# soniareilly/HPCClassMultigridProject

Measured on AMD Instinct MI355X. Metric: V-cycle grid-point-updates/sec at N=16384; achieved HBM GB/s vs peak, higher is better.
Workload: dtype f64

## Files before the change

hpcclassmultigridproject_amd/csrc/kernels.h:

```cpp
#pragma once
#include <hip/hip_runtime.h>

namespace mgx {

struct Coef {
    double rr, nu, h, dgs, drhs, rdgs;
    unsigned dsign;
    double g, gn, c2;
    int fm;
};
Coef make_coef(double k, double nu, double h, int fm = 0);

long tower_pitch(long n);

void launch_raw_gs_colour(double *u, const double *rhs, const double *v1, const double *v2,
                          long n, Coef c, int colour, hipStream_t s);
void launch_raw_residual(double *res, const double *u, const double *rhs, const double *v1,
                         const double *v2, long n, Coef c, hipStream_t s);
void launch_raw_rhs(double *rhs, const double *u, const double *v1, const double *v2, long n,
                    Coef c, hipStream_t s);
void launch_raw_prolongation(double *up, const double *u, long n, hipStream_t s);
void launch_injection(double *dst, long dst_pitch, const double *src, long src_pitch, long m,
                      hipStream_t s);
void launch_injection_rows(double *dst, long dst_pitch, const double *src, long src_pitch,
// ... 25 lines not shown
constexpr int kCoarseLdsMaxN = 64;
constexpr int kCoarseLdsNP = kCoarseLdsMaxN + 1;

struct CoarseFuse {
    double *u = nullptr;
    const double *rhs = nullptr, *v1 = nullptr, *v2 = nullptr;
    long n = 0, pitch = 0;
    Coef c{};
    double tol = 0.0;
    int maxit = 0, zero_first = 0, reps = 0;
    double *stats = nullptr;
    int on = 0;
};

struct SmoothArgs {
    const double *uin;
    double *uout;
    const double *rhs, *v1, *v2;
    long n, pitch;
    Coef c;
    const double *uc;
    double *rhsc;
    long pitchc;
    double *partials;
    double *norm_out;
    double *rhs_out = nullptr;
    const double *zrow = nullptr;
    int vz = 0x7fffffff;
    VGen vg{};
    bool norm_sqrt = true;
    bool norm_accumulate = false;
    int ra = 0, rb = -1, lo = 0, hi = -1;
    CoarseFuse cf{};
};
int launch_smooth(const SmoothArgs &a, int sweeps, int mode, hipStream_t s);
int launch_smooth_wpair(const SmoothArgs &a, int nsmooth, hipStream_t s);
bool smooth_generates_velocity(const SmoothArgs &a, int sweeps, int mode);

struct XArgs {
    const double *uin = nullptr;
    double *upost = nullptr, *upre = nullptr;
    const double *rhs = nullptr, *v1 = nullptr, *v2 = nullptr;
    const double *uc = nullptr;
    long pitchc = 0;
    double *rhsc = nullptr;
    double *partials = nullptr, *norm_out = nullptr;
    long n = 0, pitch = 0;
    Coef c{};
    bool store_post = true;
    bool norm_sqrt = true;
    bool norm_accumulate = false;
    int ra = 0, rb = -1, lo = 0, hi = -1;
    int min_rows = 64;
    double *rhs_next = nullptr, *norm2_out = nullptr;
    const double *sa1 = nullptr, *sb1 = nullptr, *sa2 = nullptr, *sb2 = nullptr;
    int band = 0, phase = 0, partials_done = 0;
    bool pin = false, pout = false;
};
int launch_xsmooth(const XArgs &a, int sweeps, hipStream_t s);
bool xpack_supported(long n, double dgs);
void launch_xexpand(const XArgs &a, const double *packed, double *out, hipStream_t s);
bool xstep_supported(long n);
void set_xfast(long v);
long get_xfast();
void set_march_tile_rows(long v);
long get_march_tile_rows();
void set_xtile_max_rows(long v);
long get_xtile_max_rows();
// ... 39 lines not shown
```

hpcclassmultigridproject_amd/csrc/mgx.hip:

```cpp
#include <hip/hip_runtime.h>

#include <algorithm>
#include <cmath>
#include <cstdint>
#include <cstdio>
#include <cstring>
#include <mutex>
#include <string>
#include <vector>

#include "ctx.h"
#include "diag.h"
#include "sepvel.h"
#include "source.h"
#include "vfactor.h"

namespace mgxi {

thread_local std::string g_err;

long g_sep_velocity = 1;

bool factor_velocity(const double *v1, const double *v2, long n, long r0, long rows, double smin,
                     std::vector<double> &a1, std::vector<double> &b1, std::vector<double> &a2,
// ... 78 lines not shown
    return MGX_OK;
}

hipEvent_t take_event(mgx_ctx *c) {
    if (!c->pool.empty()) {
        hipEvent_t e = c->pool.back();
        c->pool.pop_back();
        return e;
    }
    hipEvent_t e = nullptr;
    if (hipEventCreate(&e) != hipSuccess) return nullptr;
    return e;
}

int prof_flush(mgx_ctx *c) {
    if (c->pending.empty()) return MGX_OK;
    HIPCHK(hipStreamSynchronize(c->stream));
    for (auto &r : c->pending) {
        float ms = 0.f;
        HIPCHK(hipEventSynchronize(r.e1));
        HIPCHK(hipEventElapsedTime(&ms, r.e0, r.e1));
        int lvl = r.level < 0 ? 0 : (r.level > 63 ? 63 : r.level);
        c->sum_ms[r.kind][lvl] += ms;
        c->sum_bytes[r.kind][lvl] += r.bytes;
        c->sum_cbytes[r.kind][lvl] += r.cbytes;
        c->count[r.kind][lvl] += 1;
        c->pool.push_back(r.e0);
        c->pool.push_back(r.e1);
    }
    c->pending.clear();
    return MGX_OK;
}

int materialize(mgx_ctx *c, int l) {
    Level &L = c->lv[l];
    if (!L.zero) return MGX_OK;
    HIPCHK(hipMemsetAsync(L.U(), 0, sizeof(double) * L.pitch * (L.n + 1), c->stream));
    L.zero = false;
    return MGX_OK;
}

int op_prolong_add(mgx_ctx *c, int l);
int op_restrict(mgx_ctx *c, int l);
long g_vgen = 1;
static mgx::VGen level_vgen(const mgx_ctx *c, int l) {
    mgx::VGen g;
    g.a = c->vga;
    g.b1 = c->lv[0].sb1;
    g.b2 = c->lv[0].sb2;
    g.l = l;
    g.strided = c->opt.tower_mode == MGX_TOWER_CORRECT ? 1 : 0;
    return g;
}
long g_coarse_fuse = 1;
int op_coarse(mgx_ctx *c, int l, int reps);
static bool coarse_fusable(const mgx_ctx *c, int l) {
    return g_coarse_fuse && !c->dist && c->opt.smoother == 0 && c->opt.nsmooth >= 1 &&
           l == c->L - 1 && l >= 2 && c->lv[l].zero &&
           c->lv[l].n <= mgx::kCoarseLdsMaxN && mgx::get_coarse_lds() &&
           c->lv[l - 1].n <= mgx::get_tile_max_n();
}
static int flush_coarse(mgx_ctx *c) {
    if (c->cf_level < 0) return MGX_OK;
    const int l = c->cf_level;
    c->cf_level = -1;
    return op_coarse(c, l, c->cf_reps);
}
static int check_coarse_rhs(const mgx::SmoothArgs &A, int mode) {
    if (A.cf.on && (mode & mgx::kModeRestrict) && A.rhsc == A.cf.rhs)
        return fail(MGX_E_INTERNAL, "fused coarsest solve reads the rhs its pass restricts into");
    return MGX_OK;
}
static bool take_coarse(mgx_ctx *c, int l, mgx::SmoothArgs &A) {
    if (c->cf_level != l + 1) return false;
    Level &Cl = c->lv[l + 1];
    A.cf.u = Cl.U();
    A.cf.rhs = Cl.rhs;
    A.cf.v1 = Cl.v1;
    A.cf.v2 = Cl.v2;
    A.cf.n = Cl.n;
    A.cf.pitch = Cl.pitch;
    A.cf.c = Cl.coef;
    A.cf.tol = c->opt.coarse_tol;
    A.cf.maxit = c->opt.coarse_maxit;
    A.cf.zero_first = Cl.zero ? 1 : 0;
    A.cf.reps = c->cf_reps;
    A.cf.stats = c->dscal + 2;
    A.cf.on = 1;
    return true;
}
static void took_coarse(mgx_ctx *c, int l) {
    c->cf_level = -1;
    c->lv[l + 1].zero = false;
}

int op_smooth(mgx_ctx *c, int l, int sweeps, bool prolong, bool restrict_, bool norm,
              bool *fused_norm) {
    Level &L = c->lv[l];
    if (fused_norm) *fused_norm = false;
    if (c->opt.smoother == 0 && sweeps > 0) {
        const int fuse = std::max(1, std::min(c->opt.fuse, mgx::kSmoothMaxSweeps));
        int done = 0;
        while (done < sweeps) {
            const int k = std::min(sweeps - done, fuse);
            const bool first = done == 0, last = done + k == sweeps;
            const bool pr = prolong && first && !L.zero;
            const bool rs = restrict_ && last;
            const bool nm = norm && last && !rs;
            const bool cfuse = pr && c->cf_level == l + 1;
            if (pr && !cfuse) CHK(materialize(c, l + 1));
            int mode = 0;
            if (L.zero) mode |= mgx::kModeZero;
            if (pr) mode |= mgx::kModeProlong;
            if (rs) mode |= mgx::kModeRestrict;
            if (nm) mode |= mgx::kModeNorm;
            mgx::SmoothArgs A{};
            A.uin = L.u[L.cur];
            A.uout = L.u[L.nxt()];
            A.rhs = L.rhs;
            A.v1 = L.v1;
            A.v2 = L.v2;
            A.zrow = c->zrow;
            A.vz = L.vz;
            if (L.vgen && g_vgen) A.vg = level_vgen(c, l);
            A.n = L.n;
            A.pitch = L.pitch;
            A.c = L.coef;
            if (pr || rs) {
                Level &Cl = c->lv[l + 1];
                A.uc = Cl.U();
                A.rhsc = Cl.rhs;
                A.pitchc = Cl.pitch;
            }
            A.partials = c->partials;
            A.norm_out = c->dscal;
            if (cfuse) take_coarse(c, l, A);
            double bytes = 40.0 * k * L.M();
            int kind = MGX_K_GS;
            if (pr) {
                bytes += 32.0 * L.M() + 8.0 * c->lv[l + 1].M();
                kind = MGX_K_PSMOOTH;
            }
            if (rs) bytes += 40.0 * L.M() + 24.0 * c->lv[l + 1].M();
            if (nm) bytes += 48.0 * L.M();
            const bool vgu = mgx::smooth_generates_velocity(A, k, mode);
            const double cbytes = 8.0 * (((mode & mgx::kModeZero) ? 2.0 : 3.0) * L.M() +
                                         (vgu ? 0.0 : 2.0 * L.Mv()) +
                                         ((pr ? 1 : 0) + (rs ? 1 : 0)) * c->lv[l + 1].M());
            int blocks = 0;
            CHK(check_coarse_rhs(A, mode));
            const size_t before = c->pending.size();
            CHK(launch(c, kind, l, bytes, cbytes,
                       [&] { blocks = mgx::launch_smooth(A, k, mode, c->stream); }));
            if (blocks < 0) unlaunch(c, before);
            if (blocks == -4 && cfuse) {
                A.cf = mgx::CoarseFuse{};
                CHK(flush_coarse(c));
                A.uc = c->lv[l + 1].U();
                CHK(launch(c, kind, l, bytes, cbytes,
                           [&] { blocks = mgx::launch_smooth(A, k, mode, c->stream); }));
            } else if (cfuse) {
                took_coarse(c, l);
            }
            if (blocks < 0) return fail(MGX_E_ARG, "launch_smooth: unsupported sweeps/mode");
            L.cur = L.nxt();
            L.packed[L.cur] = false;
            L.zero = false;
            if (rs) c->lv[l + 1].zero = true;
            if (nm && fused_norm) *fused_norm = true;
            done += k;
        }
        if (prolong && L.zero) CHK(op_prolong_add(c, l));
        return MGX_OK;
    }
    if (prolong) CHK(op_prolong_add(c, l));
    for (int k = 0; k < sweeps; ++k) {
        if (c->opt.smoother == 2) {
            const bool z = L.zero;
            CHK(launch(c, MGX_K_GS, l, 40.0 * L.M(), [&] {
                mgx::launch_gs_sweep(L.u[L.cur], L.u[L.nxt()], L.rhs, L.v1, L.v2, L.n, L.pitch,
                                     L.coef, z, c->stream);
            }));
            L.cur = L.nxt();
            L.zero = false;
        } else {
            CHK(materialize(c, l));
            CHK(launch(c, MGX_K_GS, l, 40.0 * L.M(), [&] {
                mgx::launch_gs_colour(L.U(), L.rhs, L.v1, L.v2, L.n, L.pitch, L.coef, 0,
                                      c->stream);
                mgx::launch_gs_colour(L.U(), L.rhs, L.v1, L.v2, L.n, L.pitch, L.coef, 1,
                                      c->stream);
            }));
        }
    }
    if (restrict_) CHK(op_restrict(c, l));
    return MGX_OK;
}

int op_gs(mgx_ctx *c, int l, int sweeps) {
// ... 16 lines not shown
    }));
    return read_norm(c, norm);
}

int op_restrict(mgx_ctx *c, int l) {
    CHK(materialize(c, l));
    Level &F = c->lv[l], &C = c->lv[l + 1];
    CHK(launch(c, MGX_K_RESTRICT, l, 40.0 * F.M() + 24.0 * C.M(), 32.0 * F.M() + 8.0 * C.M(), [&] {
        mgx::launch_residual_restrict(F.U(), F.rhs, F.v1, F.v2, F.n, F.pitch, F.coef, C.rhs,
                                      C.pitch, c->stream);
    }));
    C.zero = true;
    return MGX_OK;
}

int op_prolong_add(mgx_ctx *c, int l) {
    CHK(flush_coarse(c));
    CHK(materialize(c, l));
    CHK(materialize(c, l + 1));
    Level &F = c->lv[l], &C = c->lv[l + 1];
    CHK(launch(c, MGX_K_PROLONG, l, 32.0 * F.M() + 8.0 * C.M(), 16.0 * F.M() + 8.0 * C.M(), [&] {
        mgx::launch_prolong_add(F.U(), F.pitch, C.U(), C.pitch, C.n, c->stream);
    }));
    return MGX_OK;
}

long g_wpair = 1;
int op_wpair(mgx_ctx *c, int l, bool *done) {
    *done = false;
    Level &L = c->lv[l], &Cl = c->lv[l + 1];
    const int k = c->opt.nsmooth;
    if (!g_wpair || c->opt.smoother != 0 || k < 1 || k > 3 || c->opt.fuse < k || L.zero)
        return MGX_OK;
    if (c->cf_level == l + 1 && !Cl.rhs_alt) CHK(flush_coarse(c));
    const bool cfuse = c->cf_level == l + 1;
    if (Cl.zero && !cfuse) return MGX_OK;
    mgx::SmoothArgs A{};
    A.uin = L.u[L.cur];
    A.uout = L.u[L.nxt()];
    A.rhs = L.rhs;
    A.v1 = L.v1;
    A.v2 = L.v2;
    A.n = L.n;
    A.pitch = L.pitch;
    A.c = L.coef;
    A.uc = Cl.U();
    A.rhsc = cfuse ? Cl.rhs_alt : Cl.rhs;
    A.pitchc = Cl.pitch;
    A.partials = c->partials;
    A.norm_out = c->dscal;
    if (cfuse) take_coarse(c, l, A);
    CHK(check_coarse_rhs(A, mgx::kModeProlong | mgx::kModeRestrict));
    const double bytes = (32.0 + 40.0 * k) * L.M() + 8.0 * Cl.M() + (40.0 * k + 40.0) * L.M() +
                         24.0 * Cl.M();
    const double cbytes = 8.0 * (3.0 * L.M() + 2.0 * L.Mv() + 2.0 * Cl.M());
    int blocks = 0;
    const size_t before = c->pending.size();
    CHK(launch(c, MGX_K_PSMOOTH, l, bytes, cbytes,
               [&] { blocks = mgx::launch_smooth_wpair(A, k, c->stream); }));
    if (blocks < 0) unlaunch(c, before);
    if (blocks == -4) return flush_coarse(c);
    if (blocks < 0) return MGX_OK;
    if (cfuse) {
        took_coarse(c, l);
        std::swap(Cl.rhs, Cl.rhs_alt);
    }
// ... 227 lines not shown
                                  c->stream));
            HIPCHK(hipMemcpyAsync(c->hscal + 6, c->dscal + 6, sizeof(double),
                                  hipMemcpyDeviceToHost, c->stream));
            HIPCHK(hipStreamSynchronize(c->stream));
            *norm = c->hscal[0];
            c->step_res0 = c->hscal[6];
            c->step_spec = true;
            return MGX_OK;
        }
        if (c->post_only) {
            bool fused = false;
            CHK(op_expand(c));
            CHK(op_smooth(c, 0, c->opt.nsmooth, true, false, true, &fused));
            L.spec = -1;
            return fused ? read_norm(c, norm) : op_residual_norm(c, 0, norm);
        }
        CHK(op_cross(c, store_post));
        return read_norm(c, norm);
    }
    if (l == 0) drop_spec(c);
    bool have_norm = false;
    bool pre_done = false;
    for (int sh = 0; sh < (l == c->L - 1 ? 1 : c->opt.shape); ++sh) {
        const bool last = sh == c->opt.shape - 1;
        if (l == c->L - 1) {
            if (coarse_fusable(c, l)) {
                c->cf_level = l;
                c->cf_reps = c->opt.shape;
            } else {
                CHK(op_coarse(c, l, c->opt.shape));
            }
        } else {
            if (!pre_done)
                CHK(op_smooth(c, l, c->opt.nsmooth, false, true, false, nullptr));
            pre_done = false;
            CHK(op_vcycle(c, l + 1));
            if (!last) {
                bool fused = false;
                CHK(op_wpair(c, l, &fused));
                if (fused) {
                    pre_done = true;
                    continue;
                }
            }
            CHK(op_smooth(c, l, c->opt.nsmooth, true, false, norm && last,
                          &have_norm));
            CHK(flush_coarse(c));
        }
    }
    if (norm) {
        if (have_norm)
            CHK(read_norm(c, norm));
        else
            CHK(op_residual_norm(c, l, norm));
    }
    return MGX_OK;
}

long g_source_sv = 1;

static mgxsrc::SrcArgs source_args(mgx_ctx *c, bool norm, double *cbytes) {
    Level &L = c->lv[0];
    mgxsrc::SrcArgs A;
    A.rhs = L.rhs;
    A.u = L.U();
    A.v1 = L.v1;
    A.v2 = L.v2;
// ... 1404 lines not shown
        mgxi::g_dist_local_side = value;
        return MGX_OK;
    }
    if (!strcmp(key, "coarse_fuse")) {
        if (value != 0 && value != 1) return fail(MGX_E_ARG, "coarse_fuse must be 0 or 1");
        mgxi::g_coarse_fuse = value;
        return MGX_OK;
    }
    if (!strcmp(key, "wpair")) {
        if (value != 0 && value != 1) return fail(MGX_E_ARG, "wpair must be 0 or 1");
        mgxi::g_wpair = value;
        return MGX_OK;
    }
    if (!strcmp(key, "dist_comm_chain")) {
        if (value != 0 && value != 1) return fail(MGX_E_ARG, "dist_comm_chain must be 0 or 1");
        mgxi::g_dist_comm_chain = value;
        return MGX_OK;
    }
    if (!strcmp(key, "dist_min_rows")) {
        if (value < 16 || (value & 1)) return fail(MGX_E_ARG, "dist_min_rows must be even, >= 16");
        mgxi::g_dist_min_rows = value;
        return MGX_OK;
    }
    if (!strcmp(key, "xfast")) {
        if (value != 0 && value != 1) return fail(MGX_E_ARG, "xfast must be 0 or 1");
        mgx::set_xfast(value);
        return MGX_OK;
    }
    if (!strcmp(key, "xpack")) {
        if (value < 0 || value > 2) return fail(MGX_E_ARG, "xpack must be 0, 1 or 2");
        mgxi::g_xpack = value;
        return MGX_OK;
    }
    if (!strcmp(key, "tile32_min_n")) {
        if (value < 0) return fail(MGX_E_ARG, "tile32_min_n must be >= 0");
        mgx::set_tile32_min_n(value);
        return MGX_OK;
    }
    if (!strcmp(key, "tile_xcd")) {
        if (value != 0 && value != 1) return fail(MGX_E_ARG, "tile_xcd must be 0 or 1");
        mgx::set_tile_xcd(value);
        return MGX_OK;
    }
    if (!strcmp(key, "march_order")) {
        if (value < 0 || value > 3) return fail(MGX_E_ARG, "march_order must be 0..3");
        mgx::set_march_order(value);
        return MGX_OK;
    }
    if (!strcmp(key, "march_min_rows")) {
        if (value < 8) return fail(MGX_E_ARG, "march_min_rows must be >= 8");
        mgx::set_march_min_rows(value);
        return MGX_OK;
    }
    if (!strcmp(key, "xtile_max_rows")) {
        if (value < 0) return fail(MGX_E_ARG, "xtile_max_rows must be >= 0");
        mgx::set_xtile_max_rows(value);
        return MGX_OK;
    }
    if (!strcmp(key, "step_cross")) {
        if (value != 0 && value != 1) return fail(MGX_E_ARG, "step_cross must be 0 or 1");
        g_step_cross = value;
        return MGX_OK;
    }
    if (!strcmp(key, "post_only")) {
        if (value < -1) return fail(MGX_E_ARG, "post_only must be >= -1");
        mgxi::g_post_only = value;
// ... 66 lines not shown
        return MGX_OK;
    }
    if (!strcmp(key, "cross_cycle")) {
        mgxi::cross_cycle_on();
        *value = mgxi::g_cross_cycle;
        return MGX_OK;
    }
    if (!strcmp(key, "dist_overlap")) {
        *value = mgxi::g_dist_overlap;
        return MGX_OK;
    }
    if (!strcmp(key, "dist_local_side")) {
        *value = mgxi::g_dist_local_side;
        return MGX_OK;
    }
    if (!strcmp(key, "dist_comm_chain")) {
        *value = mgxi::g_dist_comm_chain;
        return MGX_OK;
    }
    if (!strcmp(key, "coarse_fuse")) {
        *value = mgxi::g_coarse_fuse;
        return MGX_OK;
    }
    if (!strcmp(key, "wpair")) {
        *value = mgxi::g_wpair;
        return MGX_OK;
    }
    if (!strcmp(key, "dist_min_rows")) {
        *value = mgxi::g_dist_min_rows;
        return MGX_OK;
    }
    if (!strcmp(key, "xpack")) {
        *value = mgxi::g_xpack;
        return MGX_OK;
    }
    if (!strcmp(key, "xfast")) {
        *value = mgx::get_xfast();
        return MGX_OK;
    }
    if (!strcmp(key, "tile32_min_n")) {
        *value = mgx::get_tile32_min_n();
        return MGX_OK;
    }
    if (!strcmp(key, "tile_xcd")) {
        *value = mgx::get_tile_xcd();
        return MGX_OK;
    }
    if (!strcmp(key, "march_order")) {
        *value = mgx::get_march_order();
        return MGX_OK;
    }
    if (!strcmp(key, "march_min_rows")) {
        *value = mgx::get_march_min_rows();
        return MGX_OK;
    }
    if (!strcmp(key, "xtile_max_rows")) {
        *value = mgx::get_xtile_max_rows();
        return MGX_OK;
    }
    if (!strcmp(key, "step_cross")) {
        *value = g_step_cross;
        return MGX_OK;
    }
    if (!strcmp(key, "post_only")) {
        *value = mgxi::g_post_only;
        return MGX_OK;
// ... 102 lines not shown
```

hpcclassmultigridproject_amd/csrc/wsmooth.hip:

```cpp
#include "stencil.h"

#include <type_traits>

namespace mgx {
namespace {

template <int K, int MODE>
struct SmoothCfg {
    static constexpr bool ZERO = (MODE & 1) != 0;
    static constexpr bool PROL = (MODE & 2) != 0;
    static constexpr bool REST = (MODE & 4) != 0;
    static constexpr bool NORM = (MODE & 8) != 0;
    static constexpr int S = 2 * K;
    static constexpr int E = S + ((REST || NORM) ? 1 : 0);
    static constexpr int H = (E + 1) / 2;
    static constexpr int NR = E + 3;
    static constexpr int NS = S + 2;
};

template <int K, int MODE>
struct WCfg {
    static constexpr bool ZERO = (MODE & 1) != 0;
    static constexpr bool PROL = (MODE & 2) != 0;
    static constexpr bool REST = (MODE & 4) != 0;
    static constexpr bool NORM = (MODE & 8) != 0;
    static constexpr bool RHSN = (MODE & 16) != 0;
    static constexpr int S = 2 * K;
    static constexpr int E = S + ((REST || NORM) ? 1 : 0);
    static constexpr int H = (E + 1) / 2;
    static constexpr int NR = S + 4;
    static constexpr int W = 2 * (64 - 2 * H);
    static constexpr int TOP = E + NR + S + 2, BOT = E + 4;
#ifndef MGX_WMINB
#define MGX_WMINB 1
#endif
    static constexpr int MINB = MGX_WMINB;
};

#ifndef MGX_WRV
#define MGX_WRV 4
#endif
#ifndef MGX_WU
#define MGX_WU 2
#endif


template <int WPB, int K, int MODE, bool G, bool PD = false, bool FM = false, bool VG = false>
__global__ __launch_bounds__(64 * WPB, (WCfg<K, MODE>::MINB)) void k_wsmooth(
    const double *__restrict__ uin, double *__restrict__ uout, const double *__restrict__ rhs,
    const double *__restrict__ v1, const double *__restrict__ v2, const double *__restrict__ uc,
    long pitchc, double *__restrict__ rhsc, double *__restrict__ partials, int n, long pitch,
    MarchRegions reg, long units_per_wg, Coef c, int lo, int hi, double *__restrict__ rhs_out,
    const double *__restrict__ zrow, int vz, VGen vg) {
    using C = WCfg<K, MODE>;
    __shared__ double2 vgl[VG ? 64 * WPB * 6 : 1];
    constexpr int S = C::S, E = C::E, H = C::H, NR = C::NR, W = C::W;
    constexpr int WRV = C::RHSN ? (MGX_WRV > 4 ? MGX_WRV : 4) : MGX_WRV;
    static_assert(WRV >= 2 && WRV <= NR - S + 1, "rhs/v prefetch distance");
    constexpr int WU = MGX_WU < NR - 3 ? MGX_WU : NR - 3;
    static_assert(WU >= 1 && WU <= NR - 3, "u prefetch distance");
    const int l = threadIdx.x & 63;
    const int wv = threadIdx.x >> 6;
    long start, end;
    march_units(reg, WPB, units_per_wg, start, end);
    const int nc = n >> 1;
    const double hh = c.h * 0.5;
    double acc = 0.0;
    const int ip = (int)pitch, ipc = (int)pitchc;
    auto rowoff = [](int r, int p) { return (long)r * (long)p; };
    int a = 0, b = 0;
    auto rowin = [&](int r) { return (unsigned)(r - a) < (unsigned)(b - a); };

    while (start < end) {
        int strip;
        region_segment(reg, WPB, wv, start, end, strip, a, b);
        start += b - a;
        if (__builtin_amdgcn_readfirstlane(strip) < 0) continue;

        const int j0 = strip * W;
        const int c0 = j0 - 2 * H + 2 * l;
        const bool act = c0 >= 0 && c0 <= n;
        const bool keep = act && l >= H && l < 64 - H;
        const bool in0 = act && c0 >= 1 && c0 <= n - 1;
        const bool in1 = act && c0 + 1 <= n - 1;
        VGCol g0{}, g1{};
        constexpr int NT = 64 * WPB;
        const int lb = threadIdx.x;
        if constexpr (VG) {
            g0 = vg_col(c0, n, vg.l, vg.strided);
            g1 = vg_col(c0 + 1, n, vg.l, vg.strided);
            vgl[lb + 0 * NT] = make_double2(vg.b1[g0.chi], vg.b2[g0.chi]);
            vgl[lb + 1 * NT] = make_double2(vg.b1[g0.clo], vg.b2[g0.clo]);
            vgl[lb + 2 * NT] = make_double2(0.0, 0.0);
            vgl[lb + 3 * NT] = make_double2(vg.b1[g1.chi], vg.b2[g1.chi]);
            vgl[lb + 4 * NT] = make_double2(vg.b1[g1.clo], vg.b2[g1.clo]);
            vgl[lb + 5 * NT] = make_double2(0.0, 0.0);
        }

        struct UPre {
            double2 X;
            double q00, q01, q10, q11;
        };
        UPre up[NR];
#pragma unroll
        for (int q = 0; q < NR; ++q) up[q] = UPre{make_double2(0.0, 0.0), 0.0, 0.0, 0.0, 0.0};
        const int cl = min(max(c0, 0), (int)pitch - 2);
        const int jl = cl >> 1;
        const int j1 = (jl + 1 <= nc) ? 1 : 0;
        auto load_u = [&](int R, UPre &u, const bool odd) {
            if (C::ZERO) return;
            const int Rc = min(max(R, lo), hi);
            u.X = ld2((uin + rowoff(Rc, ip)) + cl);
            if (C::PROL) {
                const double *p0 = (uc + rowoff(Rc >> 1, ipc)) + jl;
                u.q00 = p0[0];
                u.q01 = p0[j1];
                if (odd) {
                    const int o1 = (Rc & 1) ? ipc : 0;
                    u.q10 = p0[o1];
                    u.q11 = p0[o1 + j1];
                }
            }
        };
        auto make_u = [&](int R, const UPre &u, const bool odd) {
            double2 v = u.X;
            if (C::ZERO) v = make_double2(0.0, 0.0);
            if (C::PROL) {
                double2 pr;
                const double q01 = (!G || j1) ? u.q01 : 0.0;
                const double q11 = (!G || j1) ? u.q11 : 0.0;
                if (!odd) {
                    pr.x = u.q00;
                    pr.y = (u.q00 + q01) / 2;
                } else {
                    pr.x = (u.q00 + u.q10) / 2;
                    pr.y = (u.q00 + u.q10 + q01 + q11) / 4;
                }
                const bool on = !G || (act && R >= 0 && R <= n);
                v.x = on ? v.x + pr.x : v.x;
                v.y = on ? v.y + pr.y : v.y;
            }
            return v;
        };
        auto load_rv = [&](int R, RowData &d) {
            const int Rc = min(max(R, lo), hi);
            const long o = rowoff(Rc, ip);
            if (!C::RHSN) d.r = ld2((rhs + o) + cl);
            if constexpr (VG) {
                d.x = vg.a[vg_row(g0, Rc, vg_state(g0, Rc), vg.l, n << vg.l)];
                d.y = vg.a[vg_row(g1, Rc, vg_state(g1, Rc), vg.l, n << vg.l)];
                return;
            }
            const bool z = Rc >= vz;
            d.x = ld2((z ? zrow : v1 + o) + cl);
            d.y = ld2((z ? zrow : v2 + o) + cl);
        };
        auto scale_rv = [&](RowData &d, const int R) {
            if constexpr (VG) {
                const int Rc = min(max(R, lo), hi);
// ... 135 lines not shown
                            else if (WH)
                                ur[iR].x = div_diag<PD>(d.r.x - k.cn.x * ur[iN].x -
                                                            cg.rr * (cg.nu - d.y.x) * uW -
                                                            k.cs.x * ur[iS].x -
                                                            cg.rr * (d.y.x + cg.nu) * ur[iR].y,
                                                        c);
                            else
                                ur[iR].x = gs_point_t<PD>(d.r.x, d.x.x, d.y.x, ur[iN].x, uW,
                                                          ur[iS].x, ur[iR].y, cg);
                        }
                    } else {
                        const double uE = dpp_shl1(ur[iR].x);
                        if (!G || (inr && in1)) {
                            if (FM && WH)
                                ur[iR].y = fm_upd2(d.r.y, k.cn.y, ur[iN].y, k.cw.y, ur[iR].x,
                                                   ur[iS].y, uE, cg);
                            else if (FM)
                                ur[iR].y = fm_upd_t(d.r.y, d.x.y, d.y.y, ur[iN].y, ur[iR].x,
                                                    ur[iS].y, uE, cg);
                            else if (WH)
                                ur[iR].y = div_diag<PD>(d.r.y - k.cn.y * ur[iN].y -
                                                            cg.rr * (cg.nu - d.y.y) * ur[iR].x -
                                                            k.cs.y * ur[iS].y -
                                                            cg.rr * (d.y.y + cg.nu) * uE,
                                                        c);
                            else
                                ur[iR].y = gs_point_t<PD>(d.r.y, d.x.y, d.y.y, ur[iN].y, ur[iR].x,
                                                          ur[iS].y, uE, cg);
                        }
                    }
                }
                {
                    const int ro = s + 2 - S;
                    st2_if(uout + rowoff(ro, ip), c0, rowin(ro) && keep,
                           ur[(p + 2 - S + 2 * NR) % NR]);
                }
                if (C::REST || C::NORM) {
                    const int r = s + 1 - S;
                    const int iR = (p + 1 - S + 2 * NR) % NR;
                    const int iN = (p - S + 2 * NR) % NR;
                    const int iS = (p + 2 - S + 2 * NR) % NR;
                    const RowData &d = rd[iR];
                    const double uW = dpp_shr1(ur[iR].y);
                    auto rx = [&]() {
                        if (WH) return res_cx(iR, iN, iS, uW);
                        if (FM)
                            return fm_res_t(d.r.x, d.x.x, d.y.x, ur[iR].x, ur[iN].x, uW, ur[iS].x,
                                            ur[iR].y, c);
                        return res_point_t(d.r.x, d.x.x, d.y.x, ur[iR].x, ur[iN].x, uW, ur[iS].x,
                                           ur[iR].y, c);
                    };
                    if (C::REST) {
                        if (((p + 1 - S) & 1) == 0 && rowin(r) && keep &&
                            (!G || (r >= 1 && r <= n - 2 && in0 && c0 <= n - 2))) {
                            const double res = rx();
                            (rhsc + rowoff(r >> 1, ipc))[c0 >> 1] = res;
                        }
                    } else {
                        const double uE = dpp_shl1(ur[iR].x);
                        auto ry = [&]() {
                            if (WH) return res_cy(iR, iN, iS, uE);
                            if (FM)
                                return fm_res_t(d.r.y, d.x.y, d.y.y, ur[iR].y, ur[iN].y, ur[iR].x,
                                                ur[iS].y, uE, c);
                            return res_point_t(d.r.y, d.x.y, d.y.y, ur[iR].y, ur[iN].y, ur[iR].x,
                                               ur[iS].y, uE, c);
                        };
                        if (!G) {
// ... 180 lines not shown
        const int b = q;
        st2(uout + gi * pitch + gj, make_double2(p0[b], p1[b]));
        if (C::REST || C::NORM) {
            const bool in0 = gi >= 1 && gi <= n - 1 && gj >= 1 && gj <= n - 1;
            const bool in1 = gi >= 1 && gi <= n - 1 && gj + 1 <= n - 1;
            if (C::REST) {
                if (!(gi & 1) && in0 && gi <= n - 2 && gj <= n - 2)
                    rhsc[(gi >> 1) * pitchc + (gj >> 1)] =
                        tres(f0[m], x0[m], y0[m], p0[b], p1[b - HW], p1[b - 1], p1[b + HW],
                                  p1[b], c);
            } else {
                if (in0) {
                    const double res = tres(f0[m], x0[m], y0[m], p0[b], p1[b - HW],
                                                 p1[b - 1], p1[b + HW], p1[b], c);
                    acc += res * res;
                }
                if (in1) {
                    const double res = tres(f1[m], x1[m], y1[m], p1[b], p0[b - HW],
                                                 p0[b], p0[b + HW], p0[b + 1], c);
                    acc += res * res;
                }
            }
        }
    }
    if (C::NORM) {
        __shared__ double red_lds[T::THREADS / 64];
        const double tot = block_sum(acc, red_lds);
        if (t == 0) partials[bid] = tot;
    }
}

}

template <int WPB, int K, int MODE, bool G, bool PD, bool FM, bool VG>
static int wsmooth_launch_pd(const SmoothArgs &A, const MarchRegions &reg, double *partials,
                             long max_wgs, hipStream_t s) {
    const long total = reg.pre[reg.count];
    if (total <= 0) return 0;
    static int slots = 0;
    if (!slots) {
        int dev = 0, cus = 0, per = 0;
        (void)hipGetDevice(&dev);
        (void)hipDeviceGetAttribute(&cus, hipDeviceAttributeMultiprocessorCount, dev);
        (void)hipOccupancyMaxActiveBlocksPerMultiprocessor(&per, k_wsmooth<WPB, K, MODE, G, PD, FM, VG>,
                                                           64 * WPB, 0);
        slots = std::max(1, cus) * std::max(1, per);
    }
    long upw;
    MarchRegions r;
    const unsigned grid = plan_march(reg, WPB, slots, get_march_min_rows(), max_wgs,
                                     WCfg<K, MODE>::E + WCfg<K, MODE>::NR / 2, upw, r);
    MGX_LAUNCH((k_wsmooth<WPB, K, MODE, G, PD, FM, VG>), dim3(grid), dim3(64 * WPB), s, A.uin,
               A.uout, A.rhs, A.v1, A.v2, A.uc, A.pitchc, A.rhsc, partials, (int)A.n, A.pitch, r,
               upw, A.c, A.lo, A.hi, A.rhs_out, A.zrow ? A.zrow : A.v1,
               A.zrow ? A.vz : 0x7fffffff, A.vg);
    return (int)grid * WPB;
}
template <int WPB, int K, int MODE, bool G, bool VG = false>
static int wsmooth_launch(const SmoothArgs &A, const MarchRegions &reg, double *partials,
                          long max_wgs, hipStream_t s) {
    if (A.c.fm)
        return wsmooth_launch_pd<WPB, K, MODE, G, false, true, VG>(A, reg, partials, max_wgs, s);
    if (A.c.dgs > 0)
        return wsmooth_launch_pd<WPB, K, MODE, G, true, false, VG>(A, reg, partials, max_wgs, s);
    return wsmooth_launch_pd<WPB, K, MODE, G, false, false, VG>(A, reg, partials, max_wgs, s);
}

template <int WPB, int K, int MODE>
static int smooth_winst(const SmoothArgs &A, hipStream_t s) {
    using C = WCfg<K, MODE>;
    MarchRegions inner, edge;
    march_regions<WPB>(A.n, C::W, C::H, A.ra, A.rb, C::TOP, C::BOT, false, inner, edge);
    if constexpr (K == 3 && (MODE == (kModeZero | kModeRestrict) || MODE == kModeProlong ||
                             MODE == kModeRestrict))
        if (A.vg.a) return wsmooth_launch<WPB, K, MODE, true, true>(A, edge, A.partials,
                                                                     kNormBlocks / WPB, s);
    return wsmooth_launch<WPB, K, MODE, true>(A, edge, A.partials, kNormBlocks / WPB, s);
}

long g_tile_max_n = 1024;
void set_tile_max_n(long v) { g_tile_max_n = v; }
long get_tile_max_n() { return g_tile_max_n; }
long g_tile32_min_n = 2048;
void set_tile32_min_n(long v) { g_tile32_min_n = v; }
long get_tile32_min_n() { return g_tile32_min_n; }
long g_tile_xcd = 1;
void set_tile_xcd(long v) { g_tile_xcd = v; }
long get_tile_xcd() { return g_tile_xcd; }

template <int K, int MODE, int TRV>
static int smooth_tile_rows(const SmoothArgs &A, hipStream_t s) {
    using T = TileCfg<K, MODE, TRV>;
    const long n = A.n;
    const int tiles_x = (int)((n + 1 + T::TC - 1) / T::TC);
    const int tiles_y = (int)((A.rb - A.ra + T::TR - 1) / T::TR);
    const long grid = (long)tiles_x * tiles_y;
    if ((MODE & 8) && grid > kNormBlocks) return -1;
    if (A.c.fm)
        MGX_LAUNCH((k_smooth_tile<K, MODE, TRV, true>), dim3((unsigned)grid), dim3(T::THREADS), s,
                   A.uin, A.uout, A.rhs, A.v1, A.v2, A.uc, A.pitchc, A.rhsc, A.partials, (int)n,
                   A.pitch, tiles_x, A.c, A.ra, A.rb, A.lo, A.hi, g_tile_xcd ? 1 : 0, A.cf);
    else
        MGX_LAUNCH((k_smooth_tile<K, MODE, TRV, false>), dim3((unsigned)grid), dim3(T::THREADS), s,
                   A.uin, A.uout, A.rhs, A.v1, A.v2, A.uc, A.pitchc, A.rhsc, A.partials, (int)n,
                   A.pitch, tiles_x, A.c, A.ra, A.rb, A.lo, A.hi, g_tile_xcd ? 1 : 0, A.cf);
// ... 6 lines not shown
        if (A.n >= g_tile32_min_n) return smooth_tile_rows<K, MODE, 32>(A, s);
    return smooth_tile_rows<K, MODE, 16>(A, s);
}

long g_march_tile_rows = 16;
void set_march_tile_rows(long v) { g_march_tile_rows = v; }
long get_march_tile_rows() { return g_march_tile_rows; }

template <int K, int MODE>
static bool smooth_as_tiles(const SmoothArgs &A) {
    bool tile = A.n <= g_tile_max_n && !(MODE & 16);
    if (!tile && !(MODE & 16)) {
        constexpr int W4 = WCfg<K, MODE>::W * 4;
        static int slots = 0;
        if (!slots) {
            int dev = 0, cus = 0, per = 0;
            (void)hipGetDevice(&dev);
            (void)hipDeviceGetAttribute(&cus, hipDeviceAttributeMultiprocessorCount, dev);
            (void)hipOccupancyMaxActiveBlocksPerMultiprocessor(&per, k_wsmooth<4, K, MODE, true>,
                                                               256, 0);
            slots = std::max(1, cus) * std::max(1, per);
        }
        const long groups = (A.n + 1 + W4 - 1) / W4;
        tile = groups * (A.rb - A.ra) < (long)slots * g_march_tile_rows;
    }
    return tile;
}

template <int K, int MODE>
static int smooth_block(const SmoothArgs &A, hipStream_t s) {
    const bool tile = smooth_as_tiles<K, MODE>(A);
    const bool fused = A.cf.on && (MODE & kModeProlong) && A.cf.n <= kCoarseLdsMaxN;
    if (A.cf.on && !fused) return -4;
    if (tile) {
        const int g = smooth_tile_inst<K, MODE>(A, s);
        if (g > 0) return g;
    }
    if (fused) return -4;
    return smooth_winst<4, K, MODE>(A, s);
}

template <int K>
static int smooth_k(const SmoothArgs &A, int mode, hipStream_t s) {
    switch (mode) {
        case 0: return smooth_block<K, 0>(A, s);
        case 1: return smooth_block<K, 1>(A, s);
        case 2: return smooth_block<K, 2>(A, s);
        case 4: return smooth_block<K, 4>(A, s);
        case 5: return smooth_block<K, 5>(A, s);
        case 8: return smooth_block<K, 8>(A, s);
        case 9: return smooth_block<K, 9>(A, s);
        case 10: return smooth_block<K, 10>(A, s);
        case 20: return smooth_block<K, 20>(A, s);
        default: return -1;
    }
}

bool smooth_generates_velocity(const SmoothArgs &A0, int sweeps, int mode) {
    if (!A0.vg.a || sweeps != 3) return false;
    SmoothArgs A = A0;
    if (A.rb < 0) {
        A.ra = 0;
        A.rb = (int)A.n + 1;
    }
    if (mode == (kModeZero | kModeRestrict)) return !smooth_as_tiles<3, kModeZero | kModeRestrict>(A);
    if (mode == kModeProlong) return !smooth_as_tiles<3, kModeProlong>(A);
    if (mode == kModeRestrict) return !smooth_as_tiles<3, kModeRestrict>(A);
    return false;
}

int launch_smooth_wpair(const SmoothArgs &A0, int nsmooth, hipStream_t s) {
    SmoothArgs A = A0;
    if (A.rb < 0) {
        A.ra = 0;
        A.rb = (int)A.n + 1;
        A.lo = 0;
        A.hi = (int)A.n;
    }
    if (A.ra & 1) return -1;
    if (A.cf.on && A.cf.n > kCoarseLdsMaxN) return -4;
    constexpr int M = kModeProlong | kModeRestrict;
    switch (nsmooth) {
        case 1:
            if (!smooth_as_tiles<1, M>(A)) return -1;
            return smooth_tile_rows<2, M, 16>(A, s);
        case 2:
            if (!smooth_as_tiles<2, M>(A)) return -1;
            return smooth_tile_rows<4, M, 16>(A, s);
        case 3:
            if (!smooth_as_tiles<3, M>(A)) return -1;
            return smooth_tile_rows<6, M, 16>(A, s);
        default: return -1;
    }
}

int launch_smooth(const SmoothArgs &A0, int sweeps, int mode, hipStream_t s) {
    SmoothArgs A = A0;
    if (A.rb < 0) {
        A.ra = 0;
        A.rb = (int)A.n + 1;
// ... 18 lines not shown
```

Measured before the change: 114.8 billion.

## Store half-packed pre-smoothed u between pre and post smoothing passes

After the zero-start pre-smoothing pass with restriction, the smoother writes only the one colour per row that is nonzero into a half-pitch packed layout. The post-smoothing prolongation pass reads that packed array and rebuilds the full row in registers, cutting write and read traffic on u by half. Anywhere else that needs full u calls a new expand step (op_wexpand) that re-runs the zero smoother. This adds template variants, packed-state bookkeeping on each level and a new wpack knob, which defaults to enabling packing only for the fm coefficient path. The risk is extra expansion launches when the packed state has to be materialised.

```diff
diff --git a/hpcclassmultigridproject_amd/csrc/kernels.h b/hpcclassmultigridproject_amd/csrc/kernels.h
--- a/hpcclassmultigridproject_amd/csrc/kernels.h
+++ b/hpcclassmultigridproject_amd/csrc/kernels.h
@@ -81,8 +81,10 @@
     bool norm_accumulate = false;
     int ra = 0, rb = -1, lo = 0, hi = -1;
     CoarseFuse cf{};
+    bool pin = false, pout = false;
 };
 int launch_smooth(const SmoothArgs &a, int sweeps, int mode, hipStream_t s);
+bool smooth_packs(const SmoothArgs &a, int sweeps);
 int launch_smooth_wpair(const SmoothArgs &a, int nsmooth, hipStream_t s);
 bool smooth_generates_velocity(const SmoothArgs &a, int sweeps, int mode);
 
diff --git a/hpcclassmultigridproject_amd/csrc/mgx.hip b/hpcclassmultigridproject_amd/csrc/mgx.hip
--- a/hpcclassmultigridproject_amd/csrc/mgx.hip
+++ b/hpcclassmultigridproject_amd/csrc/mgx.hip
@@ -134,11 +134,13 @@
     return MGX_OK;
 }
 
+static int op_wexpand(mgx_ctx *c, int l);
 int materialize(mgx_ctx *c, int l) {
     Level &L = c->lv[l];
-    if (!L.zero) return MGX_OK;
+    if (!L.zero) return op_wexpand(c, l);
     HIPCHK(hipMemsetAsync(L.U(), 0, sizeof(double) * L.pitch * (L.n + 1), c->stream));
     L.zero = false;
+    if (l >= 1) L.packed[L.cur] = false;
     return MGX_OK;
 }
 
@@ -196,10 +198,41 @@
     c->lv[l + 1].zero = false;
 }
 
+long g_wpack = 2;
+static bool wpack_on(const Level &L) {
+    return g_wpack == 1 || g_wpack == 3 || (g_wpack == 2 && L.coef.fm);
+}
+
+static int op_wexpand(mgx_ctx *c, int l) {
+    Level &L = c->lv[l];
+    if (l < 1 || !L.packed[L.cur]) return MGX_OK;
+    const int k = c->opt.nsmooth;
+    mgx::SmoothArgs A{};
+    A.uin = L.u[L.cur];
+    A.uout = L.u[L.cur];
+    A.rhs = L.rhs;
+    A.v1 = L.v1;
+    A.v2 = L.v2;
+    A.zrow = c->zrow;
+    A.vz = L.vz;
+    A.n = L.n;
+    A.pitch = L.pitch;
+    A.c = L.coef;
+    A.partials = c->partials;
+    A.norm_out = c->dscal;
+    int blocks = 0;
+    CHK(launch(c, MGX_K_GS, l, 40.0 * k * L.M(), 8.0 * (2.0 * L.M() + 2.0 * L.Mv()),
+               [&] { blocks = mgx::launch_smooth(A, k, mgx::kModeZero, c->stream); }));
+    if (blocks < 0) return fail(MGX_E_INTERNAL, "op_wexpand: unsupported sweeps");
+    L.packed[L.cur] = false;
+    return MGX_OK;
+}
+
 int op_smooth(mgx_ctx *c, int l, int sweeps, bool prolong, bool restrict_, bool norm,
-              bool *fused_norm) {
+              bool *fused_norm, bool pack_out = false) {
     Level &L = c->lv[l];
     if (fused_norm) *fused_norm = false;
+    if (c->opt.smoother != 0 || sweeps <= 0) CHK(op_wexpand(c, l));
     if (c->opt.smoother == 0 && sweeps > 0) {
         const int fuse = std::max(1, std::min(c->opt.fuse, mgx::kSmoothMaxSweeps));
         int done = 0;
@@ -237,6 +270,14 @@
             A.partials = c->partials;
             A.norm_out = c->dscal;
             if (cfuse) take_coarse(c, l, A);
+            const bool pk_form = l >= 1 && !c->dist && first && last && (k == 2 || k == 3) &&
+                                 mgx::smooth_packs(A, k);
+            if (l >= 1 && L.packed[L.cur] &&
+                (!(pk_form && mode == mgx::kModeProlong) || g_wpack == 3))
+                CHK(op_wexpand(c, l));
+            A.pin = l >= 1 && L.packed[L.cur];
+            A.pout = pack_out && pk_form && wpack_on(L) &&
+                     mode == (mgx::kModeZero | mgx::kModeRestrict);
             double bytes = 40.0 * k * L.M();
             int kind = MGX_K_GS;
             if (pr) {
@@ -248,7 +289,8 @@
             const bool vgu = mgx::smooth_generates_velocity(A, k, mode);
             const double cbytes = 8.0 * (((mode & mgx::kModeZero) ? 2.0 : 3.0) * L.M() +
                                          (vgu ? 0.0 : 2.0 * L.Mv()) +
-                                         ((pr ? 1 : 0) + (rs ? 1 : 0)) * c->lv[l + 1].M());
+                                         ((pr ? 1 : 0) + (rs ? 1 : 0)) * c->lv[l + 1].M() -
+                                         0.5 * L.M() * ((A.pin ? 1 : 0) + (A.pout ? 1 : 0)));
             int blocks = 0;
             CHK(check_coarse_rhs(A, mode));
             const size_t before = c->pending.size();
@@ -265,8 +307,9 @@
                 took_coarse(c, l);
             }
             if (blocks < 0) return fail(MGX_E_ARG, "launch_smooth: unsupported sweeps/mode");
+            if (l >= 1) L.packed[L.cur] = false;
             L.cur = L.nxt();
-            L.packed[L.cur] = false;
+            L.packed[L.cur] = A.pout;
             L.zero = false;
             if (rs) c->lv[l + 1].zero = true;
             if (nm && fused_norm) *fused_norm = true;
@@ -349,6 +392,7 @@
     const int k = c->opt.nsmooth;
     if (!g_wpair || c->opt.smoother != 0 || k < 1 || k > 3 || c->opt.fuse < k || L.zero)
         return MGX_OK;
+    if (L.packed[L.cur]) return MGX_OK;
     if (c->cf_level == l + 1 && !Cl.rhs_alt) CHK(flush_coarse(c));
     const bool cfuse = c->cf_level == l + 1;
     if (Cl.zero && !cfuse) return MGX_OK;
@@ -642,7 +686,8 @@
             }
         } else {
             if (!pre_done)
-                CHK(op_smooth(c, l, c->opt.nsmooth, false, true, false, nullptr));
+                CHK(op_smooth(c, l, c->opt.nsmooth, false, true, false, nullptr,
+                              l >= 1));
             pre_done = false;
             CHK(op_vcycle(c, l + 1));
             if (!last) {
@@ -2113,6 +2158,11 @@
         mgxi::g_xpack = value;
         return MGX_OK;
     }
+    if (!strcmp(key, "wpack")) {
+        if (value < 0 || value > 3) return fail(MGX_E_ARG, "wpack must be 0, 1, 2 or 3");
+        mgxi::g_wpack = value;
+        return MGX_OK;
+    }
     if (!strcmp(key, "tile32_min_n")) {
         if (value < 0) return fail(MGX_E_ARG, "tile32_min_n must be >= 0");
         mgx::set_tile32_min_n(value);
@@ -2245,6 +2295,10 @@
     }
     if (!strcmp(key, "xpack")) {
         *value = mgxi::g_xpack;
+        return MGX_OK;
+    }
+    if (!strcmp(key, "wpack")) {
+        *value = mgxi::g_wpack;
         return MGX_OK;
     }
     if (!strcmp(key, "xfast")) {
diff --git a/hpcclassmultigridproject_amd/csrc/wsmooth.hip b/hpcclassmultigridproject_amd/csrc/wsmooth.hip
--- a/hpcclassmultigridproject_amd/csrc/wsmooth.hip
+++ b/hpcclassmultigridproject_amd/csrc/wsmooth.hip
@@ -4,6 +4,14 @@
 
 namespace mgx {
 namespace {
+
+__device__ __forceinline__ void st1s_if(double *row, int col, bool on, double v) {
+#if MGX_NTST
+    if (on) __builtin_nontemporal_store(v, row + col);
+#else
+    if (on) row[col] = v;
+#endif
+}
 
 template <int K, int MODE>
 struct SmoothCfg {
@@ -45,7 +53,8 @@
 #endif
 
 
-template <int WPB, int K, int MODE, bool G, bool PD = false, bool FM = false, bool VG = false>
+template <int WPB, int K, int MODE, bool G, bool PD = false, bool FM = false, bool VG = false,
+          int PK = 0>
 __global__ __launch_bounds__(64 * WPB, (WCfg<K, MODE>::MINB)) void k_wsmooth(
     const double *__restrict__ uin, double *__restrict__ uout, const double *__restrict__ rhs,
     const double *__restrict__ v1, const double *__restrict__ v2, const double *__restrict__ uc,
@@ -67,6 +76,11 @@
     const double hh = c.h * 0.5;
     double acc = 0.0;
     const int ip = (int)pitch, ipc = (int)pitchc;
+    const int ihp = ip >> 1;
+    static_assert(PK == 0 || (G && !C::NORM && !C::RHSN &&
+                              (PK == 1 ? (C::ZERO && C::REST && !C::PROL)
+                                       : (C::PROL && !C::ZERO && !C::REST))),
+                  "packed rows: the guarded ZERO|REST pass writes them, the PROL pass reads them");
     auto rowoff = [](int r, int p) { return (long)r * (long)p; };
     int a = 0, b = 0;
     auto rowin = [&](int r) { return (unsigned)(r - a) < (unsigned)(b - a); };
@@ -110,7 +124,10 @@
         auto load_u = [&](int R, UPre &u, const bool odd) {
             if (C::ZERO) return;
             const int Rc = min(max(R, lo), hi);
-            u.X = ld2((uin + rowoff(Rc, ip)) + cl);
+            if (PK == 2)
+                u.X.x = ((uin + rowoff(Rc, ihp)) + (cl >> 1))[0];
+            else
+                u.X = ld2((uin + rowoff(Rc, ip)) + cl);
             if (C::PROL) {
                 const double *p0 = (uc + rowoff(Rc >> 1, ipc)) + jl;
                 u.q00 = p0[0];
@@ -125,6 +142,7 @@
         auto make_u = [&](int R, const UPre &u, const bool odd) {
             double2 v = u.X;
             if (C::ZERO) v = make_double2(0.0, 0.0);
+            if (PK == 2) v = odd ? make_double2(u.X.x, 0.0) : make_double2(0.0, u.X.x);
             if (C::PROL) {
                 double2 pr;
                 const double q01 = (!G || j1) ? u.q01 : 0.0;
@@ -326,8 +344,12 @@
                 }
                 {
                     const int ro = s + 2 - S;
-                    st2_if(uout + rowoff(ro, ip), c0, rowin(ro) && keep,
-                           ur[(p + 2 - S + 2 * NR) % NR]);
+                    const double2 uf = ur[(p + 2 - S + 2 * NR) % NR];
+                    if (PK == 1)
+                        st1s_if(uout + rowoff(ro, ihp), c0 >> 1, rowin(ro) && keep,
+                                (p & 1) ? uf.x : uf.y);
+                    else
+                        st2_if(uout + rowoff(ro, ip), c0, rowin(ro) && keep, uf);
                 }
                 if (C::REST || C::NORM) {
                     const int r = s + 1 - S;
@@ -574,7 +596,7 @@
 
 }
 
-template <int WPB, int K, int MODE, bool G, bool PD, bool FM, bool VG>
+template <int WPB, int K, int MODE, bool G, bool PD, bool FM, bool VG, int PK>
 static int wsmooth_launch_pd(const SmoothArgs &A, const MarchRegions &reg, double *partials,
                              long max_wgs, hipStream_t s) {
     const long total = reg.pre[reg.count];
@@ -584,28 +606,28 @@
         int dev = 0, cus = 0, per = 0;
         (void)hipGetDevice(&dev);
         (void)hipDeviceGetAttribute(&cus, hipDeviceAttributeMultiprocessorCount, dev);
-        (void)hipOccupancyMaxActiveBlocksPerMultiprocessor(&per, k_wsmooth<WPB, K, MODE, G, PD, FM, VG>,
-                                                           64 * WPB, 0);
+        (void)hipOccupancyMaxActiveBlocksPerMultiprocessor(
+            &per, k_wsmooth<WPB, K, MODE, G, PD, FM, VG, PK>, 64 * WPB, 0);
         slots = std::max(1, cus) * std::max(1, per);
     }
     long upw;
     MarchRegions r;
     const unsigned grid = plan_march(reg, WPB, slots, get_march_min_rows(), max_wgs,
                                      WCfg<K, MODE>::E + WCfg<K, MODE>::NR / 2, upw, r);
-    MGX_LAUNCH((k_wsmooth<WPB, K, MODE, G, PD, FM, VG>), dim3(grid), dim3(64 * WPB), s, A.uin,
+    MGX_LAUNCH((k_wsmooth<WPB, K, MODE, G, PD, FM, VG, PK>), dim3(grid), dim3(64 * WPB), s, A.uin,
                A.uout, A.rhs, A.v1, A.v2, A.uc, A.pitchc, A.rhsc, partials, (int)A.n, A.pitch, r,
                upw, A.c, A.lo, A.hi, A.rhs_out, A.zrow ? A.zrow : A.v1,
                A.zrow ? A.vz : 0x7fffffff, A.vg);
     return (int)grid * WPB;
 }
-template <int WPB, int K, int MODE, bool G, bool VG = false>
+template <int WPB, int K, int MODE, bool G, bool VG = false, int PK = 0>
 static int wsmooth_launch(const SmoothArgs &A, const MarchRegions &reg, double *partials,
                           long max_wgs, hipStream_t s) {
     if (A.c.fm)
-        return wsmooth_launch_pd<WPB, K, MODE, G, false, true, VG>(A, reg, partials, max_wgs, s);
+        return wsmooth_launch_pd<WPB, K, MODE, G, false, true, VG, PK>(A, reg, partials, max_wgs, s);
     if (A.c.dgs > 0)
-        return wsmooth_launch_pd<WPB, K, MODE, G, true, false, VG>(A, reg, partials, max_wgs, s);
-    return wsmooth_launch_pd<WPB, K, MODE, G, false, false, VG>(A, reg, partials, max_wgs, s);
+        return wsmooth_launch_pd<WPB, K, MODE, G, true, false, VG, PK>(A, reg, partials, max_wgs, s);
+    return wsmooth_launch_pd<WPB, K, MODE, G, false, false, VG, PK>(A, reg, partials, max_wgs, s);
 }
 
 template <int WPB, int K, int MODE>
@@ -613,6 +635,20 @@
     using C = WCfg<K, MODE>;
     MarchRegions inner, edge;
     march_regions<WPB>(A.n, C::W, C::H, A.ra, A.rb, C::TOP, C::BOT, false, inner, edge);
+    constexpr int PK = (K < 2) ? 0
+                       : MODE == (kModeZero | kModeRestrict) ? 1
+                       : MODE == kModeProlong ? 2 : 0;
+    const bool pk = PK == 1 ? A.pout : A.pin;
+    if ((A.pin || A.pout) && (PK == 0 || !pk)) return -1;
+    if constexpr (PK != 0) {
+        if (pk) {
+            if constexpr (K == 3)
+                if (A.vg.a) return wsmooth_launch<WPB, K, MODE, true, true, PK>(
+                                A, edge, A.partials, kNormBlocks / WPB, s);
+            return wsmooth_launch<WPB, K, MODE, true, false, PK>(A, edge, A.partials,
+                                                                 kNormBlocks / WPB, s);
+        }
+    }
     if constexpr (K == 3 && (MODE == (kModeZero | kModeRestrict) || MODE == kModeProlong ||
                              MODE == kModeRestrict))
         if (A.vg.a) return wsmooth_launch<WPB, K, MODE, true, true>(A, edge, A.partials,
@@ -685,6 +721,7 @@
     const bool tile = smooth_as_tiles<K, MODE>(A);
     const bool fused = A.cf.on && (MODE & kModeProlong) && A.cf.n <= kCoarseLdsMaxN;
     if (A.cf.on && !fused) return -4;
+    if ((A.pin || A.pout) && tile) return -1;
     if (tile) {
         const int g = smooth_tile_inst<K, MODE>(A, s);
         if (g > 0) return g;
@@ -719,6 +756,17 @@
     if (mode == (kModeZero | kModeRestrict)) return !smooth_as_tiles<3, kModeZero | kModeRestrict>(A);
     if (mode == kModeProlong) return !smooth_as_tiles<3, kModeProlong>(A);
     if (mode == kModeRestrict) return !smooth_as_tiles<3, kModeRestrict>(A);
+    return false;
+}
+
+bool smooth_packs(const SmoothArgs &A0, int sweeps) {
+    SmoothArgs A = A0;
+    if (A.rb >= 0) return false;
+    A.ra = 0;
+    A.rb = (int)A.n + 1;
+    constexpr int PRE = kModeZero | kModeRestrict, POST = kModeProlong;
+    if (sweeps == 2) return !smooth_as_tiles<2, PRE>(A) && !smooth_as_tiles<2, POST>(A);
+    if (sweeps == 3) return !smooth_as_tiles<3, PRE>(A) && !smooth_as_tiles<3, POST>(A);
     return false;
 }
 
```

After: 119.0 billion (median of 6 runs). 1.04x the previous value.
